# happyxtt/CNNs_SLFP_quantization

Hardware: AMD Instinct MI355X
Metric: images/sec at batch 256, MobileNetV1 SLFP<3,4> ImageNet-224; % HBM roofline (higher is better)
Workload: dtype f32 (1x1 contraction: fp16 MFMA operands, f32 accumulate); 1 GPU; mobilenetv1_imagenet224: all 27 Conv2d_Q layers, SLFP<3,4> Qbits=8, NHWC, batch 256 per GPU as 2 concurrent image groups of 128 on 2 HIP streams, inputs resident in HBM; batch_per_gpu=256, global_batch=256, parallelism=batch-sharded x1, one-time RCCL broadcast of the u8 weight codes, pointwise_mfma=pw_mfma_f16x1

## Files before the change

cnns_slfp_quantization_amd/_lib.py:

```python
import ctypes
import os

_HERE = os.path.dirname(os.path.abspath(__file__))
LIB_PATH = os.path.join(_HERE, "libslfp_hip.so")

OK, ERR_BAD_ARG, ERR_SHAPE, ERR_UNSUPPORTED, ERR_ALIGNMENT, ERR_HIP = 0, -1, -2, -3, -4, -5
FMT_ACT8, FMT_W8, FMT_SFP7, FMT_EXT = 0, 1, 2, 4
LAYOUT_NCHW, LAYOUT_NHWC = 0, 1
BWD_DENSE = 1
MFMA_DEFAULT, MFMA_F16X1, MFMA_F16X3 = 0, 1, 3
OPT_SGD, OPT_DSGD, OPT_SSGD = 0, 1, 2
LAYEROUT_LUT_BYTES = 4928

SYMBOLS = (
    "slfp_version", "slfp_last_error", "slfp_device_count",
    "slfp_encode_f32", "slfp_decode_f32", "slfp_quantize_f32", "slfp_quantize_layerout_f32", "slfp_absmax_f32",
    "slfp_conv2d_out_shape", "slfp_conv2d_kernel_name", "slfp_conv2d_wprep_bytes",
    "slfp_conv2d_prepare_weights", "slfp_conv2d_prepare_weights_codes", "slfp_conv2d_workspace_bytes", "slfp_conv2d_fwd", "slfp_conv2d_fwd_post",
    "slfp_linear_workspace_bytes", "slfp_linear_fwd", "slfp_linear_prepare_weights", "slfp_linear_fwd_prepared",
    "slfp_nchw_to_nhwc_f32", "slfp_nhwc_to_nchw_f32", "slfp_debug_div_mismatches",
    "slfp_debug_enc_mismatches", "slfp_enc_table_ok", "slfp_dwpw_supported", "slfp_dwpw_fwd",
    "slfp_conv2d_codes_supported", "slfp_conv2d_fwd_codes", "slfp_conv2d_fwd_codes_ws", "slfp_maxpool2d_codes", "slfp_debug_code_mismatches", "slfp_debug_reload_switches",
    "slfp_debug_enc_hl_mismatches", "slfp_sgd_step_f32", "slfp_debug_dw3x3_variant", "slfp_debug_dense_variant", "slfp_debug_pw_variant",
    "slfp_conv2d_bwd_supported", "slfp_conv2d_bwd_kernel_name", "slfp_conv2d_bwd_workspace_bytes", "slfp_conv2d_bwd",
    "slfp_conv2d_bwd_supported_ex", "slfp_conv2d_bwd_kernel_name_ex", "slfp_conv2d_bwd_workspace_bytes_ex", "slfp_conv2d_bwd_ex",
    "slfp_conv2d_res_supported", "slfp_conv2d_fwd_res",
    "slfp_conv2d_codes_slice_supported", "slfp_conv2d_fwd_codes_slice", "slfp_maxpool2d_codes_ex", "slfp_maxpool2d_out_shape",
    "slfp_conv2d_entry_supported", "slfp_conv2d_fwd_entry",
    "slfp_conv2d_res_codes_supported", "slfp_conv2d_fwd_res_codes",
    "slfp_layerout_lut_classes", "slfp_layerout_lut_values", "slfp_layerout_lut_index", "slfp_conv2d_codes_lut_supported",
    "slfp_conv2d_fwd_codes_lut", "slfp_debug_layerout_lut_mismatches",
    "slfp_dwpw_codes_supported", "slfp_dwpw_fwd_codes",
    "slfp_linear_fc_supported", "slfp_linear_fc_workspace_bytes", "slfp_linear_fwd_fc", "slfp_debug_linear_fc_tiles",
    "slfp_global_avgpool_supported", "slfp_global_avgpool_f32",
    "slfp_debug_dw3x3_instance", "slfp_debug_code_relu_mismatches",
)


class ConvDesc(ctypes.Structure):
    _fields_ = [
        ("n", ctypes.c_int64), ("c_in", ctypes.c_int64), ("h", ctypes.c_int64), ("w", ctypes.c_int64),
        ("c_out", ctypes.c_int64), ("kh", ctypes.c_int64), ("kw", ctypes.c_int64),
        ("stride_h", ctypes.c_int32), ("stride_w", ctypes.c_int32), ("pad_h", ctypes.c_int32),
        ("pad_w", ctypes.c_int32), ("dil_h", ctypes.c_int32), ("dil_w", ctypes.c_int32),
        ("groups", ctypes.c_int32), ("x_layout", ctypes.c_int32), ("y_layout", ctypes.c_int32),
        ("qbits", ctypes.c_int32), ("ka", ctypes.c_float), ("kw_scale", ctypes.c_float),
        ("mfma_passes", ctypes.c_int32), ("reserved", ctypes.c_int32),
    ]


# ... 30 lines not shown
    dp = ctypes.POINTER(ConvDesc)
    sigs = {
        "slfp_version": (ci, []),
        "slfp_last_error": (ctypes.c_char_p, []),
        "slfp_device_count": (ci, []),
        "slfp_encode_f32": (ci, [vp, vp, sz, cf, ci, vp]),
        "slfp_decode_f32": (ci, [vp, vp, sz, ci, vp]),
        "slfp_quantize_f32": (ci, [vp, vp, sz, cf, ci, vp]),
        "slfp_quantize_layerout_f32": (ci, [vp, vp, sz, vp]),
        "slfp_absmax_f32": (ci, [vp, sz, vp, vp]),
        "slfp_conv2d_out_shape": (ci, [dp, ctypes.POINTER(i64), ctypes.POINTER(i64)]),
        "slfp_conv2d_kernel_name": (ctypes.c_char_p, [dp]),
        "slfp_debug_dw3x3_variant": (ctypes.c_char_p, [dp, ci]),
        "slfp_debug_dw3x3_instance": (ctypes.c_char_p, [dp, ctypes.POINTER(ConvIo), ci, ci, ci]),
        "slfp_debug_code_relu_mismatches": (ci, [cf, ci, vp, vp]),
        "slfp_debug_dense_variant": (ctypes.c_char_p, [dp, ci]),
        "slfp_debug_pw_variant": (ctypes.c_char_p, [dp, ctypes.POINTER(ConvIo), ci, ci, i64]),
        "slfp_conv2d_wprep_bytes": (sz, [dp]),
        "slfp_conv2d_prepare_weights": (ci, [dp, vp, vp, vp, vp]),
        "slfp_conv2d_prepare_weights_codes": (ci, [dp, vp, vp, vp, vp]),
        "slfp_conv2d_workspace_bytes": (sz, [dp]),
        "slfp_conv2d_fwd": (ci, [dp, vp, vp, vp, vp, vp, vp, vp]),
        "slfp_conv2d_fwd_post": (ci, [dp, vp, vp, vp, vp, vp, ci, vp, vp, vp, vp]),
        "slfp_linear_workspace_bytes": (sz, [i64, i64, i64]),
        "slfp_linear_fwd": (ci, [vp, vp, vp, vp, i64, i64, i64, cf, cf, ci, ci, vp, vp]),
        "slfp_linear_prepare_weights": (ci, [vp, vp, i64, i64, cf, ci, ci, vp]),
        "slfp_linear_fwd_prepared": (ci, [vp, vp, vp, vp, i64, i64, i64, cf, cf, ci, ci, vp]),
        "slfp_nchw_to_nhwc_f32": (ci, [vp, vp, i64, i64, i64, i64, vp]),
        "slfp_nhwc_to_nchw_f32": (ci, [vp, vp, i64, i64, i64, i64, vp]),
        "slfp_debug_div_mismatches": (ci, [cf, vp, vp]),
# ... 66 lines not shown
```

cnns_slfp_quantization_amd/csrc/conv_abi.hip:

```cpp
#include <cstring>
#include "slfp_device.hpp"
#include "slfp_codes.hpp"
#include "slfp_layerout_lut.hpp"
#include "slfp_host.hpp"

namespace slfp {

static size_t round256(size_t b) { return (b + 255) & ~(size_t)255; }

static int make_plan_core(const slfp_conv2d_desc* d, ConvPlan* plan) {
    if (!d || !plan) return fail(SLFP_ERR_BAD_ARG, "conv2d: null descriptor");
    if (d->n <= 0 || d->c_in <= 0 || d->h <= 0 || d->w <= 0 || d->c_out <= 0 || d->kh <= 0 || d->kw <= 0)
        return fail(SLFP_ERR_SHAPE, "conv2d: non-positive size");
    if (d->stride_h <= 0 || d->stride_w <= 0 || d->dil_h <= 0 || d->dil_w <= 0 || d->pad_h < 0 || d->pad_w < 0)
        return fail(SLFP_ERR_SHAPE, "conv2d: bad stride/dilation/padding");
    if (d->groups <= 0 || d->c_in % d->groups || d->c_out % d->groups)
        return fail(SLFP_ERR_SHAPE, "conv2d: groups=%d does not divide C_in=%lld / C_out=%lld", d->groups,
                    (long long)d->c_in, (long long)d->c_out);
    if (d->qbits != 8 && d->qbits != 7)
        return fail(SLFP_ERR_BAD_ARG, "conv2d: qbits must be 8 (SLFP<3,4>) or 7 (SFP<3,3>), got %d", d->qbits);
    if ((d->x_layout != SLFP_LAYOUT_NCHW && d->x_layout != SLFP_LAYOUT_NHWC) ||
        (d->y_layout != SLFP_LAYOUT_NCHW && d->y_layout != SLFP_LAYOUT_NHWC))
        return fail(SLFP_ERR_BAD_ARG, "conv2d: unknown layout");
    if (!(d->ka > 0.f) || !(d->kw_scale > 0.f)) return fail(SLFP_ERR_BAD_ARG, "conv2d: Ka and Kw must be > 0");
// ... 237 lines not shown

const char* slfp_debug_dw3x3_instance(const slfp_conv2d_desc* d, const slfp_conv2d_io* io, int has_bias, int post_flags, int has_post) {
    return dw3x3_instance(d, io, has_bias != 0, post_flags, has_post != 0);
}

const char* slfp_debug_dense_variant(const slfp_conv2d_desc* d, int x_codes) {
    ConvPlan p;
    if (make_plan(d, &p) != SLFP_OK) return "none";
    return dense_variant_name(*d, p, x_codes != 0);
}

const char* slfp_debug_pw_variant(const slfp_conv2d_desc* d, const slfp_conv2d_io* io, int has_res, int has_res_codes, int64_t y_ld) {
    return pw_variant(d, io, has_res != 0, has_res_codes != 0, y_ld);
}

size_t slfp_conv2d_wprep_bytes(const slfp_conv2d_desc* d) {
    ConvPlan p;
    if (make_plan(d, &p) != SLFP_OK) return 0;
    return p.wprep_bytes;
}

static int prepare_weights(const char* fn, const slfp_conv2d_desc* d, const void* w, void* wprep, float* weight_q_oihw, void* stream,
                           bool codes) {
    ConvPlan p;
    const int rc = make_plan(d, &p);
    if (rc != SLFP_OK) return rc;
    if (!w || !wprep) return fail(SLFP_ERR_BAD_ARG, "%s: null pointer", fn);
    if (!aligned16(wprep)) return fail(SLFP_ERR_ALIGNMENT, "%s: wprep must be 16-byte aligned", fn);
    return launch_prepare_weights(*d, p, reinterpret_cast<const float*>(w), wprep, weight_q_oihw, as_stream(stream), codes);
}
// ... 572 lines not shown
```

cnns_slfp_quantization_amd/csrc/conv_direct.hip:

```cpp
#include "slfp_device.hpp"
#include "slfp_enc.hpp"
#include "slfp_codes.hpp"
#include "slfp_layerout_lut.hpp"
#include "slfp_host.hpp"
#include "slfp_epilogue.hpp"

namespace slfp {

constexpr int kDirThreads = 256;
constexpr int kDirTH = 8, kDirTW = 8, kDirOC = 64;

struct DirParams {
    int N, H, W, C, O, KH, KW;
    int sh, sw, ph, pw, dh, dw;
    int groups, Cg, Og, Ho, Wo;
    int tiles_h, tiles_w, oc_chunks;
    int CC, IH, IW;
    ScaleDiv sd;
    float s1, s2;
    PostOp post;
    uint32_t nblocks;
};

template <int FMT>
// ... 91 lines not shown
        float* dst = y + (((size_t)n * p.Ho + goh) * p.Wo + gow) * p.O + o0;
        if (o_vec) {
            *reinterpret_cast<float4*>(dst) = make_float4(r4[0], r4[1], r4[2], r4[3]);
        } else {
#pragma unroll
            for (int r = 0; r < 4; ++r)
                if (r < n_o) dst[r] = r4[r];
        }
    }
}


constexpr int kStemTH = 8, kStemTW = 16;

struct StemParams {
    int N, H, W, C, O, KH, KW;
    int s, ph, pw;
    int Ho, Wo, tiles_h, tiles_w;
    int IH, IWC;
    int l4_shift;
    int P;
    int step_h, step_j;
    ScaleDiv sd;
    float s1, s2;
    PostOp post;
    uint32_t nblocks;
    EncArgs enc;
    EncArgsCompact enc_out;
    int sgn, fmt_out;
};

template <int FMT>
__global__ __launch_bounds__(256) void k_stem(const float* __restrict__ x, const float* __restrict__ wq,
                                              const float* __restrict__ bias, float* __restrict__ y, const StemParams p) {
    extern __shared__ __attribute__((aligned(16))) unsigned char smem[];
    uint32_t* sT = reinterpret_cast<uint32_t*>(smem);
    float* sW = reinterpret_cast<float*>(smem + 64);
    const int n_w = p.KH * p.KW * p.C * p.O;
    float* tile = sW + ((n_w + 3) & ~3);
    lut_fill<FMT>(sT);
    for (int i = threadIdx.x * 4; i < n_w; i += 256 * 4)
// ... 258 lines not shown
}

template <bool YC, bool LUTQ = false>
__global__ __launch_bounds__(256) void k_stem_mx(const float* __restrict__ x, const float* __restrict__ wq,
                                                 const float* __restrict__ bias, float* __restrict__ y, const StemParams p) {
    constexpr int KH = 3, KW = 3, C = 3, S = 2, O = 32, TH = 16;
    constexpr int IH = (TH - 1) * S + KH, IWC = ((kStemTW - 1) * S + KW) * C;
    constexpr int N_IN = IH * IWC, U = (N_IN + 255) / 256;
    typedef float f32x4m __attribute__((ext_vector_type(4)));
    __shared__ __attribute__((aligned(16))) float tile[N_IN + 1];
    __shared__ __attribute__((aligned(16))) uint32_t sT[2 * (kEncEntries + 1)];
    static_assert(!LUTQ || YC, "the table epilogue belongs to the code-writing forms");
    __shared__ __attribute__((aligned(16))) unsigned char senc[LUTQ ? kLayeroutLutBytes : (YC ? ((kEncEntries * 8 + 15) & ~15) : 16)];
    constexpr int SP = 36;
    __shared__ __attribute__((aligned(16))) float stg[YC ? 4 : 4 * 16 * SP];
    enc_fill<256>(reinterpret_cast<uint2*>(sT), p.enc);
    if constexpr (LUTQ) layerout_lut_fill<256>(senc, enc_carried_ptr(p.enc_out));
    else if constexpr (YC) enc_fill_compact<256>(reinterpret_cast<uint2*>(senc), p.enc_out);
    if (threadIdx.x == 0) tile[N_IN] = 0.f;

    uint32_t b = xcd_remap(blockIdx.x, p.nblocks);
    const int tw = b % p.tiles_w; b /= p.tiles_w;
    const int th = b % p.tiles_h; b /= p.tiles_h;
    const int n = b;
    const int h_in0 = th * TH * S - p.ph, w_in0 = tw * kStemTW * S - p.pw;

    const int lane = threadIdx.x & 63, wave = threadIdx.x >> 6;
    const int px = lane & 15, kq = lane >> 4;
    float wa[7][2];
#pragma unroll
    for (int ks = 0; ks < 7; ++ks) {
        const int k = 4 * ks + kq;
#pragma unroll
        for (int t = 0; t < 2; ++t) wa[ks][t] = k < KH * KW * C ? wq[k * O + 8 * (px >> 2) + 4 * t + (px & 3)] : 0.f;
    }
    uint32_t koff[7];
#pragma unroll
    for (int ks = 0; ks < 7; ++ks) {
        const int k = 4 * ks + kq;
        koff[ks] = (uint32_t)((k / (KW * C)) * IWC + (k % (KW * C))) * 4u;
    }
    __syncthreads();

    {
        constexpr int Q = (IWC + 1 + 3) / 4;
        constexpr int N4 = IH * Q, U4 = (N4 + 255) / 256;
        const float* xn = x + (size_t)n * p.H * p.W * C;
        const int rowf = p.W * C;
        const int s0 = w_in0 * C - 1;
        const __amdgpu_buffer_rsrc_t rs = __builtin_amdgcn_make_buffer_rsrc(const_cast<float*>(xn), 0, (uint32_t)p.H * p.W * C * 4u, 0x00020000);
        uint32_t vo[U4];
        typedef float f32x4l __attribute__((ext_vector_type(4)));
        f32x4l v[U4];
#pragma unroll
        for (int u = 0; u < U4; ++u) {
            const int idx = threadIdx.x + u * 256;
            const int ih = idx / Q, q = idx - ih * Q;
            const int gh = h_in0 + ih, f0 = s0 + 4 * q;
            const bool ok = idx < N4 && (unsigned)gh < (unsigned)p.H && f0 >= 0 && f0 < rowf;
            vo[u] = ok ? (uint32_t)(gh * rowf + f0) * 4u : 0xFFFFFFF0u;
            asm volatile("" : "+v"(vo[u]));
        }
#pragma unroll
        for (int u = 0; u < U4; ++u) v[u] = __builtin_bit_cast(f32x4l, __builtin_amdgcn_raw_buffer_load_b128(rs, vo[u], 0, 0));
        const unsigned char* tb = reinterpret_cast<const unsigned char*>(sT);
#pragma unroll
        for (int u = 0; u < U4; ++u) {
            const int idx = threadIdx.x + u * 256;
            const int ih = idx / Q, q = idx - ih * Q;
            const float4 xv = make_float4(v[u][0], v[u][1], v[u][2], v[u][3]);
            const float4 qv = enc4_f32(xv, p.enc.r1, p.enc.lo, p.enc.hi, tb);
            const float qs[4] = {qv.x, qv.y, qv.z, qv.w};
            float* trow = tile + ih * IWC + 4 * q - 1;
#pragma unroll
            for (int e = 0; e < 4; ++e)
                if (idx < N4 && 4 * q + e >= 1 && 4 * q + e - 1 < IWC) trow[e] = qs[e];
        }
    }
    __syncthreads();
// ... 100 lines not shown
    p.P = kStemTH / (groups / kStemTW);
    p.step_h = 256 / p.IWC; p.step_j = 256 % p.IWC;
    p.sd = make_scale_div(d.ka); p.s1 = plan.s1; p.s2 = plan.s2;
    const size_t n_w = (size_t)p.KH * p.KW * C * O;
    const size_t lds = 64 + (((n_w + 3) & ~(size_t)3) + (size_t)p.IH * p.IWC) * sizeof(float);
    if (lds > 64 * 1024) return 1;
    const int64_t nblocks = (int64_t)p.N * p.tiles_h * p.tiles_w;
    if (nblocks > 0x7FFFFFFF) return 1;
    p.nblocks = (uint32_t)nblocks;
    if (p.KH == 3 && p.KW == 3 && C == 3 && p.s == 2 && O == 32 && (int64_t)p.H * p.W * C < (1ll << 30)) {
        if (const EncArgs* t = act_table(d.ka, plan.fmt_act, kEncF32)) {
            p.enc = *t;
            constexpr int TH = 16;
            p.tiles_h = (int)ceil_div(p.Ho, TH);
            p.nblocks = (uint32_t)((int64_t)p.N * p.tiles_h * p.tiles_w);
            const bool mx = !switches().stem_old && (p.W * C) % 4 == 0;
            if (mx && !(io && io->y_codes)) {
                hipLaunchKernelGGL((k_stem_mx<false>), dim3(p.nblocks), dim3(256), 0, stream, x, wq_hwio, bias, y, p);
                return check_launch("slfp stem conv kernel (3x3x3 s2 -> 32, float32 MFMA)");
            }
            if (io && io->lut) {
                if (!io->y_codes || !post.scale) return fail(SLFP_ERR_BAD_ARG, "stem (codes): the table epilogue needs code output and post_scale / post_shift");
                p.enc_out.valid = 0;
                enc_carry_ptr(p.enc_out, io->lut);
                p.sgn = 1;
                p.fmt_out = io->y_fmt;
                if (mx) hipLaunchKernelGGL((k_stem_mx<true, true>), dim3(p.nblocks), dim3(256), 0, stream, x, wq_hwio, bias, y, p);
                else hipLaunchKernelGGL((k_stem_fixed<kFmtAct8, 3, 3, 3, 2, 32, true, TH, true, true>), dim3(p.nblocks), dim3(256), 0, stream, x, wq_hwio, bias, y, p);
                return check_launch("slfp stem conv kernel (3x3x3 s2 -> 32, table epilogue)");
            }
// ... 75 lines not shown
```

cnns_slfp_quantization_amd/csrc/conv_dw2.hip:

```cpp
#include <cstdlib>
#include "slfp_device.hpp"
#include "slfp_enc.hpp"
#include "slfp_host.hpp"

namespace slfp {

constexpr int kDw2Threads = 256;
constexpr int kDw2Tab = (kEncEntries * 8 + 15) & ~15;
constexpr uint32_t kOob = 0xFFFFFFF0u;

struct Dw2Params {
    int N, H, W, C, Ho, Wo;
    int tiles_h, tiles_w, cgroups;
    int pad;
    uint32_t ntiles;
    uint32_t nblocks;
    float ka, kw;
    int nt_out;
    PostOp post;
    EncArgs enc;
};

typedef float f32x4 __attribute__((ext_vector_type(4)));

__device__ __forceinline__ __amdgpu_buffer_rsrc_t make_rsrc(const void* base, uint32_t bytes) {
    return __builtin_amdgcn_make_buffer_rsrc(const_cast<void*>(base), 0, bytes, 0x00020000);
}

template <int S, int TH, int TW, bool POST>
__global__ __launch_bounds__(kDw2Threads, 4) void k_dw3x3_tile(const float* __restrict__ x, const float* __restrict__ wq,
                                                               float* __restrict__ y, const Dw2Params p) {
    constexpr int IH = (TH - 1) * S + 3, IW = (TW - 1) * S + 3;
    static_assert(IW <= 16 && IH <= 16, "halo tile is at most 16 x 16 pixel slots");
    constexpr int NI = (IH + 1) / 2;
    constexpr int ROWB = 16 * 32 * 4;

    __shared__ __attribute__((aligned(16))) unsigned char smem[kDw2Tab + 2 * NI * ROWB];
    unsigned char* tile = smem + kDw2Tab;
    enc_fill<kDw2Threads>(reinterpret_cast<uint2*>(smem), p.enc);
    const float r1 = p.enc.r1, lo = p.enc.lo, hi = p.enc.hi;

    const uint32_t lb = xcd_remap(blockIdx.x, p.nblocks);
    const int cg = (int)(lb % (uint32_t)p.cgroups);
    const uint32_t t = lb / (uint32_t)p.cgroups;

    const int c4 = threadIdx.x & 7, slot = threadIdx.x >> 3;
    const int c = cg * 32 + c4 * 4;
    const int iw = slot & 15, ihh = slot >> 4;

    f32x4 wt[9];
#pragma unroll
    for (int k = 0; k < 9; ++k) wt[k] = *reinterpret_cast<const f32x4*>(wq + (size_t)k * p.C + c);
    f32x4 psc = {1.f, 1.f, 1.f, 1.f}, psh = {0.f, 0.f, 0.f, 0.f};
    if constexpr (POST) {
        psc = *reinterpret_cast<const f32x4*>(p.post.scale + c);
        psh = *reinterpret_cast<const f32x4*>(p.post.shift + c);
    }

    const int colslot = (S == 2) ? ((iw & 1) * 8 + (iw >> 1)) : iw;
    const uint32_t lds_w = (uint32_t)((ihh * 16 + colslot) * 128 + c4 * 16);
    const bool col_live = iw < IW;
    constexpr int CW = TW > 8 ? 16 : 8, RPI = 32 / CW, NO = (TH + RPI - 1) / RPI;
    const int ow = slot & (CW - 1), ohb = slot / CW;
    const bool ocol_live = ow < TW;
    const uint32_t lds_r0 = (uint32_t)(((ohb * S) * 16 + ow) * 128 + c4 * 16);
    const uint32_t out_rel0 = (uint32_t)((ohb * p.Wo + ow) * p.C + c) * 4u;
    const uint32_t out_step = (uint32_t)(RPI * p.Wo * p.C) * 4u;
    const uint32_t img_in_bytes = (uint32_t)p.H * p.W * p.C * 4u, img_out_bytes = (uint32_t)p.Ho * p.Wo * p.C * 4u;
    const uint32_t tiles_per_img = (uint32_t)(p.tiles_h * p.tiles_w);

    const uint32_t n = t / tiles_per_img, tr = t - n * tiles_per_img;
    const int th = (int)(tr / (uint32_t)p.tiles_w), tw = (int)(tr - (uint32_t)th * p.tiles_w);

    f32x4 v[NI];
    {
        const __amdgpu_buffer_rsrc_t rs = make_rsrc(x + (size_t)n * p.H * p.W * p.C, img_in_bytes);
        const int gw = tw * TW * S - p.pad + iw;
        const int gh0 = th * TH * S - p.pad + ihh;
        const bool w_ok = col_live && (unsigned)gw < (unsigned)p.W;
        const uint32_t off0 = (uint32_t)((gh0 * p.W + gw) * p.C + c) * 4u;
        const uint32_t step = (uint32_t)(2 * p.W * p.C) * 4u;
        uint32_t voff[NI];
#pragma unroll
        for (int i = 0; i < NI; ++i) {
            bool ok = w_ok && (unsigned)(gh0 + 2 * i) < (unsigned)p.H;
            if (2 * i + 1 >= IH) ok = ok && ihh == 0;
            voff[i] = ok ? off0 + (uint32_t)i * step : kOob;
            asm volatile("" : "+v"(voff[i]));
        }
#pragma unroll
        for (int i = 0; i < NI; ++i)
            v[i] = __builtin_bit_cast(f32x4, __builtin_amdgcn_raw_buffer_load_b128(rs, voff[i], 0, (SLFP_NT_DW & 1) ? 2 : 0));
    }
    __syncthreads();

    bool any_nan = false;
#pragma unroll
    for (int i = 0; i < NI; ++i) {
        const float4 xi = make_float4(v[i][0], v[i][1], v[i][2], v[i][3]);
        any_nan |= enc_has_nan4(xi);
        *reinterpret_cast<float4*>(tile + lds_w + (uint32_t)i * 2u * ROWB) = enc4_f32_raw(xi, r1, lo, hi, smem);
    }
    if (__builtin_expect(any_nan, 0)) {
#pragma unroll
        for (int i = 0; i < NI; ++i)
#pragma unroll
            for (int e = 0; e < 4; ++e)
                if (v[i][e] != v[i][e]) reinterpret_cast<uint32_t*>(tile + lds_w + (uint32_t)i * 2u * ROWB)[e] = kBitsQNaN;
    }
// ... 51 lines not shown
    const Dw2Sel s = dw2_select(d, post);
    if (s.s == 2) return s.post ? "tile/s2/post" : "tile/s2/plain";
    return s.post ? "tile/s1/post" : "tile/s1/plain";
}

int launch_dw3x3_tile(const slfp_conv2d_desc& d, const ConvPlan& plan, const float* x, const float* wq9c,
                      const PostOp& post, float* y, hipStream_t stream) {
    Dw2Params p;
    const Dw2Sel sel = dw2_select(d, post);
    p.post = post;
    p.N = (int)d.n; p.H = (int)d.h; p.W = (int)d.w; p.C = (int)d.c_in;
    p.Ho = (int)plan.h_out; p.Wo = (int)plan.w_out;
    const int S = sel.s;
    const int TH = S == 2 ? 7 : 14, TW = TH;
    p.tiles_h = (int)ceil_div(p.Ho, TH);
    p.tiles_w = (int)ceil_div(p.Wo, TW);
    p.cgroups = p.C / 32;
    p.pad = d.pad_h;
    const int64_t ntiles = (int64_t)p.N * p.tiles_h * p.tiles_w;
    if (ntiles * p.cgroups > 0x7FFFFFFF) return fail(SLFP_ERR_UNSUPPORTED, "dw3x3: grid too large");
    p.ntiles = (uint32_t)ntiles;
    p.nblocks = (uint32_t)(ntiles * p.cgroups);
    p.ka = d.ka; p.kw = d.kw_scale;
    {
        const int64_t min_mb = switches().dw_nt_min_mb;
        p.nt_out = ((SLFP_NT_DW & 2) && (int64_t)p.N * p.Ho * p.Wo * p.C * 4 >= (min_mb << 20)) ? 1 : 0;
    }
    p.enc = *act_table(d.ka, plan.fmt_act, kEncF32);
#define SLFP_DW2(SS, TT) \
    do { if (sel.post) hipLaunchKernelGGL((k_dw3x3_tile<SS, TT, TT, true>), dim3(p.nblocks), dim3(kDw2Threads), 0, stream, x, wq9c, y, p); \
         else hipLaunchKernelGGL((k_dw3x3_tile<SS, TT, TT, false>), dim3(p.nblocks), dim3(kDw2Threads), 0, stream, x, wq9c, y, p); } while (0)
    if (S == 2) SLFP_DW2(2, 7);
    else SLFP_DW2(1, 14);
#undef SLFP_DW2
    return check_launch("slfp dw3x3 (tile) kernel");
}

// ... 2 lines not shown
```

cnns_slfp_quantization_amd/csrc/conv_dw3.hip:

```cpp
#include "slfp_device.hpp"
#include "slfp_enc.hpp"
#include "slfp_host.hpp"

namespace slfp {

constexpr int kDwrThreads = 256;
constexpr int kDwrWaves = kDwrThreads / 64;
constexpr int kDwrTab = (kEncEntries * 8 + 15) & ~15;
constexpr int kDwrTile = 7;

struct DwrParams {
    int N, H, W, C, Ho, Wo, pad;
    int cgs;
    int tiles_h, tiles_w;
    uint32_t ntasks;
    uint32_t nblocks;
    float ka, kw;
    int nt_out;
    PostOp post;
    EncArgs enc;
};

typedef float f32x4 __attribute__((ext_vector_type(4)));
typedef unsigned int u32x4r __attribute__((ext_vector_type(4)));

template <int TH, bool POST>
__global__ __launch_bounds__(kDwrThreads, 4) void k_dw3x3_rows(const float* __restrict__ x, const float* __restrict__ wq,
                                                               float* __restrict__ y, const DwrParams p) {
    constexpr int S = 2, TW = kDwrTile;
    constexpr int NR = (TH - 1) * S + 3;
    constexpr int RING = 3 + S;

    __shared__ __attribute__((aligned(16))) unsigned char smem[kDwrTab];
    enc_fill<kDwrThreads>(reinterpret_cast<uint2*>(smem), p.enc);
    const float r1 = p.enc.r1, lo = p.enc.lo, hi = p.enc.hi;

    uint32_t t = xcd_remap(blockIdx.x, p.nblocks) * kDwrWaves + (uint32_t)__builtin_amdgcn_readfirstlane((int)(threadIdx.x >> 6));
    const bool valid = t < p.ntasks;
    t = valid ? t : p.ntasks - 1;
    const int cg = (int)(t % (uint32_t)p.cgs); t /= (uint32_t)p.cgs;
    const int tw = (int)(t % (uint32_t)p.tiles_w); t /= (uint32_t)p.tiles_w;
    const int th = (int)(t % (uint32_t)p.tiles_h);
    const int n = (int)(t / (uint32_t)p.tiles_h);
    const int lane = (int)(threadIdx.x & 63), g = lane >> 3;
    const int c = cg * 32 + (lane & 7) * 4;

    f32x4 wt[9];
#pragma unroll
    for (int k = 0; k < 9; ++k) wt[k] = *reinterpret_cast<const f32x4*>(wq + (uint32_t)(k * p.C + c));
    f32x4 psc = {1.f, 1.f, 1.f, 1.f}, psh = {0.f, 0.f, 0.f, 0.f};
    if constexpr (POST) {
        psc = *reinterpret_cast<const f32x4*>(p.post.scale + c);
        psh = *reinterpret_cast<const f32x4*>(p.post.shift + c);
    }

    const uint32_t img_in = (uint32_t)(p.H * p.W * p.C) * 4u, img_out = (uint32_t)(p.Ho * p.Wo * p.C) * 4u;
    const __amdgpu_buffer_rsrc_t rs = __builtin_amdgcn_make_buffer_rsrc(const_cast<float*>(x + (size_t)n * (img_in / 4u)), 0, img_in, 0x00020000);
    const __amdgpu_buffer_rsrc_t ry = __builtin_amdgcn_make_buffer_rsrc(y + (size_t)n * (img_out / 4u), 0, img_out, 0x00020000);

    const int ih0 = valid ? th * TH * S - p.pad : -0x40000000;
    const int ow = tw * TW + g, iw0 = ow * S - p.pad;
    const uint32_t rstep = (uint32_t)(p.W * p.C) * 4u;
    const uint32_t rowb = (uint32_t)ih0 * rstep + (uint32_t)c * 4u;
    uint32_t coff[2];
    coff[0] = (unsigned)iw0 < (unsigned)p.W ? (uint32_t)(iw0 * p.C) * 4u : 0x40000000u;
    coff[1] = (g < TW && (unsigned)(iw0 + 1) < (unsigned)p.W) ? (uint32_t)((iw0 + 1) * p.C) * 4u : 0x40000000u;
    const int nb_addr = ((lane + 8) & 63) * 4;

    f32x4 win[RING][3];
    auto request = [&](const int j) {
        const uint32_t roff = (unsigned)(ih0 + j) < (unsigned)p.H ? rowb + (uint32_t)j * rstep : 0x80000000u;
#pragma unroll
        for (int k = 0; k < 2; ++k)
// ... 34 lines not shown
#pragma unroll
                for (int k = 0; k < 2; ++k)
#pragma unroll
                    for (int e = 0; e < 4; ++e)
                        if (nan_mask >> (((j - j0) * 2 + k) * 4 + e) & 1u) win[j % RING][k][e] = __uint_as_float(kBitsQNaN);
        }
#pragma unroll
        for (int j = j0; j < j0 + nj; ++j)
#pragma unroll
            for (int e = 0; e < 4; ++e)
                win[j % RING][2][e] = __int_as_float(__builtin_amdgcn_ds_bpermute(nb_addr, __float_as_int(win[j % RING][0][e])));
    };

#pragma unroll
    for (int j = 0; j < RING && j < NR; ++j) request(j);

    const int oh0 = th * TH;
    const uint32_t ostep = (uint32_t)(p.Wo * p.C) * 4u;
    const uint32_t ocol = (valid && g < TW && ow < p.Wo) ? (uint32_t)((oh0 * p.Wo + ow) * p.C + c) * 4u : 0x80000000u;

    __syncthreads();

    quantize(0, 3 - S);
#pragma unroll
    for (int r = 0; r < TH; ++r) {
        quantize(r * S + 3 - S, S);
        f32x4 acc = {0.f, 0.f, 0.f, 0.f};
#pragma unroll
        for (int kh = 0; kh < 3; ++kh) {
#pragma unroll
            for (int kw = 0; kw < 3; ++kw) {
                const f32x4 a = win[(r * S + kh) % RING][kw];
                const f32x4 w = wt[kh * 3 + kw];
#pragma unroll
                for (int e = 0; e < 4; ++e) acc[e] = fmaf(a[e], w[e], acc[e]);
            }
// ... 27 lines not shown

struct DwrSel { bool post; };
static DwrSel dwr_select(const PostOp& post) { return DwrSel{post.scale != nullptr}; }

const char* dw3x3_rows_name(const slfp_conv2d_desc& d, const ConvPlan& plan, const PostOp& post) {
    return dwr_select(post).post ? "rows/post" : "rows/plain";
}

int launch_dw3x3_rows(const slfp_conv2d_desc& d, const ConvPlan& plan, const float* x, const float* wq9c,
                      const PostOp& post, float* y, hipStream_t stream) {
    DwrParams p;
    const DwrSel sel = dwr_select(post);
    p.post = post;
    p.N = (int)d.n; p.H = (int)d.h; p.W = (int)d.w; p.C = (int)d.c_in;
    p.Ho = (int)plan.h_out; p.Wo = (int)plan.w_out; p.pad = d.pad_h;
    p.cgs = p.C / 32;
    p.tiles_h = (int)ceil_div(p.Ho, kDwrTile);
    p.tiles_w = (int)ceil_div(p.Wo, kDwrTile);
    const int64_t ntasks = (int64_t)p.N * p.tiles_h * p.tiles_w * p.cgs;
    if (ntasks > 0x7FFFFFFF) return fail(SLFP_ERR_UNSUPPORTED, "dw3x3 (rows): grid too large");
    p.ntasks = (uint32_t)ntasks;
    p.nblocks = (uint32_t)ceil_div(ntasks, kDwrWaves);
    p.ka = d.ka; p.kw = d.kw_scale;
    p.nt_out = ((SLFP_NT_DW & 2) && (int64_t)p.N * p.Ho * p.Wo * p.C * 4 >= (switches().dw_nt_min_mb << 20)) ? 1 : 0;
    p.enc = *act_table(d.ka, plan.fmt_act, kEncF32);
    if (sel.post) hipLaunchKernelGGL((k_dw3x3_rows<kDwrTile, true>), dim3(p.nblocks), dim3(kDwrThreads), 0, stream, x, wq9c, y, p);
    else hipLaunchKernelGGL((k_dw3x3_rows<kDwrTile, false>), dim3(p.nblocks), dim3(kDwrThreads), 0, stream, x, wq9c, y, p);
    return check_launch("slfp dw3x3 (rows) kernel");
}

}
```

cnns_slfp_quantization_amd/csrc/slfp_enc.hpp:

```cpp
#pragma once
#include <hip/hip_runtime.h>
#include <stdint.h>

namespace slfp {

constexpr int kEncEntries = 257;
constexpr uint32_t kEncNever = 0x7FC00000u;

constexpr int kEncF32 = 0;
constexpr int kEncF16P = 1;
constexpr int kEncF16LO = 3;

struct EncArgs {
    float r1, lo, hi;
    uint32_t valid;
    uint2 e[kEncEntries];
};

template <int NT>
__device__ __forceinline__ void enc_fill(uint2* sTab, const EncArgs& a) {
    for (int i = threadIdx.x; i < kEncEntries; i += NT) sTab[i] = a.e[i];
}

constexpr int kEncCompact = 146;
struct EncArgsCompact {
    float r1, lo, hi;
    uint32_t valid;
    uint2 e[kEncCompact];
};

inline EncArgsCompact enc_compact(const EncArgs& a) {
    EncArgsCompact c;
    c.r1 = a.r1; c.lo = a.lo; c.hi = a.hi; c.valid = a.valid;
    for (int i = 0; i < kEncCompact; ++i) c.e[i] = a.e[i < 96 ? 160 + i : i - 96];
    return c;
}
// ... 137 lines not shown
```

cnns_slfp_quantization_amd/csrc/slfp_host.hpp:

```cpp
#pragma once
#include <hip/hip_runtime.h>
#include <stdint.h>
#include <stddef.h>
#include <cmath>
#include <cstring>
#include <cstdlib>
#include "../../include/slfp.h"
#include "slfp_device.hpp"
#include "slfp_enc.hpp"

namespace slfp {

void set_error(const char* fmt, ...);
int fail(int code, const char* fmt, ...);
int check_launch(const char* what);

int raise_lds_limit(const void* fn, size_t lds_bytes);

inline hipStream_t as_stream(void* s) { return reinterpret_cast<hipStream_t>(s); }
inline bool aligned16(const void* p) { return (reinterpret_cast<uintptr_t>(p) & 15u) == 0; }
inline int64_t ceil_div(int64_t a, int64_t b) { return (a + b - 1) / b; }

inline bool scale_div_ok(float d) { return std::isfinite(d) && d >= 1e-30f && d <= 1e30f; }

// ... 125 lines not shown

bool stem_small_applicable(const slfp_conv2d_desc& d, int passes);
int stem_small_tiles(const slfp_conv2d_desc& d);
int launch_stem_small(const slfp_conv2d_desc& d, const ConvPlan& p, const float* x, const void* wblob,
                      const float* bias, const PostOp& post, float* y, hipStream_t stream);
bool stem_small_codes_applicable(const slfp_conv2d_desc& d, const ConvPlan& p, int post_flags);
int launch_stem_small_io(const slfp_conv2d_desc& d, const ConvPlan& p, const float* x, const void* wblob, const float* bias,
                         const PostOp& post, void* y_any, const CodeIo& io, hipStream_t stream);

__device__ __forceinline__ uint32_t xcd_remap(uint32_t bid, uint32_t nblocks) {
    const uint32_t xcd = bid & 7u, slot = bid >> 3;
    const uint32_t q = nblocks >> 3, r = nblocks & 7u;
    const uint32_t base = xcd < r ? xcd * (q + 1u) : r * (q + 1u) + (xcd - r) * q;
    return base + slot;
}

}
```

include/slfp.h:

```cpp
#ifndef SLFP_H_
#define SLFP_H_

#include <stddef.h>
#include <stdint.h>

#ifdef __cplusplus
extern "C" {
#endif

#define SLFP_ABI_VERSION 1

#define SLFP_OK 0
#define SLFP_ERR_BAD_ARG (-1)
#define SLFP_ERR_SHAPE (-2)
#define SLFP_ERR_UNSUPPORTED (-3)
#define SLFP_ERR_ALIGNMENT (-4)
#define SLFP_ERR_HIP (-5)

#define SLFP_FMT_ACT8 0
#define SLFP_FMT_W8 1
#define SLFP_FMT_SFP7 2
#define SLFP_FMT_EXT 4

#define SLFP_LAYOUT_NCHW 0
// ... 126 lines not shown
                             const slfp_conv2d_io* io, int has_bias, int relu);
size_t slfp_linear_fc_workspace_bytes(int64_t batch, int64_t in_f, int64_t out_f, const slfp_conv2d_io* io);
int slfp_linear_fwd_fc(const void* x, const void* wprep, const float* bias, void* y, int64_t batch, int64_t in_f,
                       int64_t out_f, float ka, float kw_scale, int qbits, int mfma_passes,
                       const slfp_conv2d_io* io, int relu, void* workspace, void* stream);
int slfp_debug_linear_fc_tiles(int n_tiles, int row_tiles);

int slfp_global_avgpool_supported(int64_t n, int64_t h, int64_t w, int64_t c, int x_layout, const slfp_conv2d_io* io);
int slfp_global_avgpool_f32(const float* x, void* y, int64_t n, int64_t h, int64_t w, int64_t c, int x_layout, int relu,
                            const slfp_conv2d_io* io, void* stream);

int slfp_debug_div_mismatches(float scale_div, unsigned long long* out2, void* stream);

int slfp_debug_enc_mismatches(float scale_div, int fmt, unsigned long long* out2, void* stream);
int slfp_debug_enc_hl_mismatches(float scale_div, int fmt, unsigned long long* out1, void* stream);
int slfp_enc_table_ok(float scale_div, int fmt);

#define SLFP_OPT_SGD 0
#define SLFP_OPT_DSGD 1
#define SLFP_OPT_SSGD 2
typedef struct slfp_sgd_hparams {
    int32_t rule, qbits;
    float lr, momentum, damp_alpha, weight_decay;
    int32_t nesterov, reserved;
} slfp_sgd_hparams;
int slfp_sgd_step_f32(const slfp_sgd_hparams* h, size_t ntensors, float* const* param, float* const* grad,
                      float* const* momentum_buf, const int64_t* numel, const uint8_t* first_step, void* stream);

int slfp_conv2d_bwd_supported(const slfp_conv2d_desc* d);
const char* slfp_conv2d_bwd_kernel_name(const slfp_conv2d_desc* d);
// ... 19 lines not shown
```

Baseline: 132,800 images/sec.

## Issue input loads before table fill; fastdiv block decode in stem and depthwise kernels

```diff
diff --git a/cnns_slfp_quantization_amd/_lib.py b/cnns_slfp_quantization_amd/_lib.py
--- a/cnns_slfp_quantization_amd/_lib.py
+++ b/cnns_slfp_quantization_amd/_lib.py
@@ -33,7 +33,7 @@
     "slfp_dwpw_codes_supported", "slfp_dwpw_fwd_codes",
     "slfp_linear_fc_supported", "slfp_linear_fc_workspace_bytes", "slfp_linear_fwd_fc", "slfp_debug_linear_fc_tiles",
     "slfp_global_avgpool_supported", "slfp_global_avgpool_f32",
-    "slfp_debug_dw3x3_instance", "slfp_debug_code_relu_mismatches",
+    "slfp_debug_dw3x3_instance", "slfp_debug_code_relu_mismatches", "slfp_debug_fastdiv_mismatches",
 )
 
 
@@ -94,6 +94,7 @@
         "slfp_debug_dw3x3_variant": (ctypes.c_char_p, [dp, ci]),
         "slfp_debug_dw3x3_instance": (ctypes.c_char_p, [dp, ctypes.POINTER(ConvIo), ci, ci, ci]),
         "slfp_debug_code_relu_mismatches": (ci, [cf, ci, vp, vp]),
+        "slfp_debug_fastdiv_mismatches": (ctypes.c_ulonglong, [ctypes.c_uint32, ctypes.c_uint32, ctypes.c_uint32]),
         "slfp_debug_dense_variant": (ctypes.c_char_p, [dp, ci]),
         "slfp_debug_pw_variant": (ctypes.c_char_p, [dp, ctypes.POINTER(ConvIo), ci, ci, i64]),
         "slfp_conv2d_wprep_bytes": (sz, [dp]),
diff --git a/cnns_slfp_quantization_amd/csrc/conv_abi.hip b/cnns_slfp_quantization_amd/csrc/conv_abi.hip
--- a/cnns_slfp_quantization_amd/csrc/conv_abi.hip
+++ b/cnns_slfp_quantization_amd/csrc/conv_abi.hip
@@ -275,6 +275,14 @@
     return pw_variant(d, io, has_res != 0, has_res_codes != 0, y_ld);
 }
 
+unsigned long long slfp_debug_fastdiv_mismatches(uint32_t d, uint32_t n_lo, uint32_t n_hi) {
+    if (d == 0 || d >= 0x80000000u || n_hi > 0x80000000u) return ~0ull;
+    const FastDiv f = make_fastdiv(d);
+    unsigned long long bad = 0;
+    for (uint32_t n = n_lo; n < n_hi; ++n) bad += fastdiv(n, f) != n / d;
+    return bad;
+}
+
 size_t slfp_conv2d_wprep_bytes(const slfp_conv2d_desc* d) {
     ConvPlan p;
     if (make_plan(d, &p) != SLFP_OK) return 0;
diff --git a/cnns_slfp_quantization_amd/csrc/conv_direct.hip b/cnns_slfp_quantization_amd/csrc/conv_direct.hip
--- a/cnns_slfp_quantization_amd/csrc/conv_direct.hip
+++ b/cnns_slfp_quantization_amd/csrc/conv_direct.hip
@@ -129,8 +129,11 @@
 constexpr int kStemTH = 8, kStemTW = 16;
 
 struct StemParams {
-    int N, H, W, C, O, KH, KW;
-    int s, ph, pw;
+    uint32_t nblocks;
+    FastDiv by_tw, by_th;
+    int H, W, ph, pw;
+    int N, C, O, KH, KW;
+    int s;
     int Ho, Wo, tiles_h, tiles_w;
     int IH, IWC;
     int l4_shift;
@@ -139,7 +142,6 @@
     ScaleDiv sd;
     float s1, s2;
     PostOp post;
-    uint32_t nblocks;
     EncArgs enc;
     EncArgsCompact enc_out;
     int sgn, fmt_out;
@@ -428,55 +430,63 @@
     __shared__ __attribute__((aligned(16))) unsigned char senc[LUTQ ? kLayeroutLutBytes : (YC ? ((kEncEntries * 8 + 15) & ~15) : 16)];
     constexpr int SP = 36;
     __shared__ __attribute__((aligned(16))) float stg[YC ? 4 : 4 * 16 * SP];
-    enc_fill<256>(reinterpret_cast<uint2*>(sT), p.enc);
-    if constexpr (LUTQ) layerout_lut_fill<256>(senc, enc_carried_ptr(p.enc_out));
-    else if constexpr (YC) enc_fill_compact<256>(reinterpret_cast<uint2*>(senc), p.enc_out);
-    if (threadIdx.x == 0) tile[N_IN] = 0.f;
-
-    uint32_t b = xcd_remap(blockIdx.x, p.nblocks);
-    const int tw = b % p.tiles_w; b /= p.tiles_w;
-    const int th = b % p.tiles_h; b /= p.tiles_h;
-    const int n = b;
+    const uint2 tab = enc_fetch<256, SLFP_ENC_KERNARG_OFF(4, StemParams)>();
+    __builtin_amdgcn_sched_barrier(0);
+
+    const uint32_t b = xcd_remap_sel(blockIdx.x, p.nblocks);
+    const uint32_t b1 = fastdiv(b, p.by_tw);
+    const int tw = (int)(b - b1 * p.by_tw.d);
+    const int n = (int)fastdiv(b1, p.by_th), th = (int)(b1 - (uint32_t)n * p.by_th.d);
     const int h_in0 = th * TH * S - p.ph, w_in0 = tw * kStemTW * S - p.pw;
 
     const int lane = threadIdx.x & 63, wave = threadIdx.x >> 6;
     const int px = lane & 15, kq = lane >> 4;
-    float wa[7][2];
-#pragma unroll
-    for (int ks = 0; ks < 7; ++ks) {
-        const int k = 4 * ks + kq;
-#pragma unroll
-        for (int t = 0; t < 2; ++t) wa[ks][t] = k < KH * KW * C ? wq[k * O + 8 * (px >> 2) + 4 * t + (px & 3)] : 0.f;
-    }
-    uint32_t koff[7];
-#pragma unroll
-    for (int ks = 0; ks < 7; ++ks) {
-        const int k = 4 * ks + kq;
-        koff[ks] = (uint32_t)((k / (KW * C)) * IWC + (k % (KW * C))) * 4u;
-    }
-    __syncthreads();
-
+
+    constexpr int Q = (IWC + 1 + 3) / 4;
+    constexpr int N4 = IH * Q, U4 = (N4 + 255) / 256;
+    typedef float f32x4l __attribute__((ext_vector_type(4)));
+    f32x4l v[U4];
     {
-        constexpr int Q = (IWC + 1 + 3) / 4;
-        constexpr int N4 = IH * Q, U4 = (N4 + 255) / 256;
         const float* xn = x + (size_t)n * p.H * p.W * C;
         const int rowf = p.W * C;
         const int s0 = w_in0 * C - 1;
         const __amdgpu_buffer_rsrc_t rs = __builtin_amdgcn_make_buffer_rsrc(const_cast<float*>(xn), 0, (uint32_t)p.H * p.W * C * 4u, 0x00020000);
         uint32_t vo[U4];
-        typedef float f32x4l __attribute__((ext_vector_type(4)));
-        f32x4l v[U4];
 #pragma unroll
         for (int u = 0; u < U4; ++u) {
             const int idx = threadIdx.x + u * 256;
             const int ih = idx / Q, q = idx - ih * Q;
             const int gh = h_in0 + ih, f0 = s0 + 4 * q;
-            const bool ok = idx < N4 && (unsigned)gh < (unsigned)p.H && f0 >= 0 && f0 < rowf;
+            const bool ok = (idx < N4) & ((unsigned)gh < (unsigned)p.H) & (f0 >= 0) & (f0 < rowf);
             vo[u] = ok ? (uint32_t)(gh * rowf + f0) * 4u : 0xFFFFFFF0u;
             asm volatile("" : "+v"(vo[u]));
         }
 #pragma unroll
         for (int u = 0; u < U4; ++u) v[u] = __builtin_bit_cast(f32x4l, __builtin_amdgcn_raw_buffer_load_b128(rs, vo[u], 0, 0));
+    }
+    __builtin_amdgcn_sched_barrier(0);
+
+    float wa[7][2];
+#pragma unroll
+    for (int ks = 0; ks < 7; ++ks) {
+        const int k = 4 * ks + kq;
+#pragma unroll
+        for (int t = 0; t < 2; ++t) wa[ks][t] = k < KH * KW * C ? wq[k * O + 8 * (px >> 2) + 4 * t + (px & 3)] : 0.f;
+    }
+    enc_store<256>(reinterpret_cast<uint2*>(sT), tab);
+    if constexpr (LUTQ) layerout_lut_fill<256>(senc, enc_carried_ptr(p.enc_out));
+    else if constexpr (YC) enc_fill_compact<256>(reinterpret_cast<uint2*>(senc), p.enc_out);
+    if (threadIdx.x == 0) tile[N_IN] = 0.f;
+    uint32_t koff[7];
+#pragma unroll
+    for (int ks = 0; ks < 7; ++ks) {
+        const int k = 4 * ks + kq;
+        koff[ks] = (uint32_t)((k / (KW * C)) * IWC + (k % (KW * C))) * 4u;
+    }
+    __syncthreads();
+    __builtin_amdgcn_sched_barrier(0);
+
+    {
         const unsigned char* tb = reinterpret_cast<const unsigned char*>(sT);
 #pragma unroll
         for (int u = 0; u < U4; ++u) {
@@ -607,6 +617,8 @@
             constexpr int TH = 16;
             p.tiles_h = (int)ceil_div(p.Ho, TH);
             p.nblocks = (uint32_t)((int64_t)p.N * p.tiles_h * p.tiles_w);
+            p.by_tw = make_fastdiv((uint32_t)p.tiles_w);
+            p.by_th = make_fastdiv((uint32_t)p.tiles_h);
             const bool mx = !switches().stem_old && (p.W * C) % 4 == 0;
             if (mx && !(io && io->y_codes)) {
                 hipLaunchKernelGGL((k_stem_mx<false>), dim3(p.nblocks), dim3(256), 0, stream, x, wq_hwio, bias, y, p);
diff --git a/cnns_slfp_quantization_amd/csrc/conv_dw2.hip b/cnns_slfp_quantization_amd/csrc/conv_dw2.hip
--- a/cnns_slfp_quantization_amd/csrc/conv_dw2.hip
+++ b/cnns_slfp_quantization_amd/csrc/conv_dw2.hip
@@ -10,11 +10,12 @@
 constexpr uint32_t kOob = 0xFFFFFFF0u;
 
 struct Dw2Params {
-    int N, H, W, C, Ho, Wo;
-    int tiles_h, tiles_w, cgroups;
-    int pad;
+    uint32_t nblocks;
+    FastDiv by_cg, by_tiles, by_tw;
+    int H, W, C, pad;
+    int N, Ho, Wo;
+    int tiles_h;
     uint32_t ntiles;
-    uint32_t nblocks;
     float ka, kw;
     int nt_out;
     PostOp post;
@@ -37,40 +38,20 @@
 
     __shared__ __attribute__((aligned(16))) unsigned char smem[kDw2Tab + 2 * NI * ROWB];
     unsigned char* tile = smem + kDw2Tab;
-    enc_fill<kDw2Threads>(reinterpret_cast<uint2*>(smem), p.enc);
-    const float r1 = p.enc.r1, lo = p.enc.lo, hi = p.enc.hi;
-
-    const uint32_t lb = xcd_remap(blockIdx.x, p.nblocks);
-    const int cg = (int)(lb % (uint32_t)p.cgroups);
-    const uint32_t t = lb / (uint32_t)p.cgroups;
+    const uint2 tab = enc_fetch<kDw2Threads, SLFP_ENC_KERNARG_OFF(3, Dw2Params)>();
+    __builtin_amdgcn_sched_barrier(0);
+
+    const uint32_t lb = xcd_remap_sel(blockIdx.x, p.nblocks);
+    const uint32_t t = fastdiv(lb, p.by_cg);
+    const int cg = (int)(lb - t * p.by_cg.d);
+    const uint32_t n = fastdiv(t, p.by_tiles), tr = t - n * p.by_tiles.d;
+    const int th = (int)fastdiv(tr, p.by_tw), tw = (int)(tr - (uint32_t)th * p.by_tw.d);
 
     const int c4 = threadIdx.x & 7, slot = threadIdx.x >> 3;
     const int c = cg * 32 + c4 * 4;
     const int iw = slot & 15, ihh = slot >> 4;
-
-    f32x4 wt[9];
-#pragma unroll
-    for (int k = 0; k < 9; ++k) wt[k] = *reinterpret_cast<const f32x4*>(wq + (size_t)k * p.C + c);
-    f32x4 psc = {1.f, 1.f, 1.f, 1.f}, psh = {0.f, 0.f, 0.f, 0.f};
-    if constexpr (POST) {
-        psc = *reinterpret_cast<const f32x4*>(p.post.scale + c);
-        psh = *reinterpret_cast<const f32x4*>(p.post.shift + c);
-    }
-
-    const int colslot = (S == 2) ? ((iw & 1) * 8 + (iw >> 1)) : iw;
-    const uint32_t lds_w = (uint32_t)((ihh * 16 + colslot) * 128 + c4 * 16);
     const bool col_live = iw < IW;
-    constexpr int CW = TW > 8 ? 16 : 8, RPI = 32 / CW, NO = (TH + RPI - 1) / RPI;
-    const int ow = slot & (CW - 1), ohb = slot / CW;
-    const bool ocol_live = ow < TW;
-    const uint32_t lds_r0 = (uint32_t)(((ohb * S) * 16 + ow) * 128 + c4 * 16);
-    const uint32_t out_rel0 = (uint32_t)((ohb * p.Wo + ow) * p.C + c) * 4u;
-    const uint32_t out_step = (uint32_t)(RPI * p.Wo * p.C) * 4u;
-    const uint32_t img_in_bytes = (uint32_t)p.H * p.W * p.C * 4u, img_out_bytes = (uint32_t)p.Ho * p.Wo * p.C * 4u;
-    const uint32_t tiles_per_img = (uint32_t)(p.tiles_h * p.tiles_w);
-
-    const uint32_t n = t / tiles_per_img, tr = t - n * tiles_per_img;
-    const int th = (int)(tr / (uint32_t)p.tiles_w), tw = (int)(tr - (uint32_t)th * p.tiles_w);
+    const uint32_t img_in_bytes = (uint32_t)p.H * p.W * p.C * 4u;
 
     f32x4 v[NI];
     {
@@ -92,7 +73,30 @@
         for (int i = 0; i < NI; ++i)
             v[i] = __builtin_bit_cast(f32x4, __builtin_amdgcn_raw_buffer_load_b128(rs, voff[i], 0, (SLFP_NT_DW & 1) ? 2 : 0));
     }
+    __builtin_amdgcn_sched_barrier(0);
+
+    f32x4 wt[9];
+#pragma unroll
+    for (int k = 0; k < 9; ++k) wt[k] = *reinterpret_cast<const f32x4*>(wq + (size_t)k * p.C + c);
+    f32x4 psc = {1.f, 1.f, 1.f, 1.f}, psh = {0.f, 0.f, 0.f, 0.f};
+    if constexpr (POST) {
+        psc = *reinterpret_cast<const f32x4*>(p.post.scale + c);
+        psh = *reinterpret_cast<const f32x4*>(p.post.shift + c);
+    }
+    enc_store<kDw2Threads>(reinterpret_cast<uint2*>(smem), tab);
+    const float r1 = p.enc.r1, lo = p.enc.lo, hi = p.enc.hi;
+
+    const int colslot = (S == 2) ? ((iw & 1) * 8 + (iw >> 1)) : iw;
+    const uint32_t lds_w = (uint32_t)((ihh * 16 + colslot) * 128 + c4 * 16);
+    constexpr int CW = TW > 8 ? 16 : 8, RPI = 32 / CW, NO = (TH + RPI - 1) / RPI;
+    const int ow = slot & (CW - 1), ohb = slot / CW;
+    const bool ocol_live = ow < TW;
+    const uint32_t lds_r0 = (uint32_t)(((ohb * S) * 16 + ow) * 128 + c4 * 16);
+    const uint32_t out_rel0 = (uint32_t)((ohb * p.Wo + ow) * p.C + c) * 4u;
+    const uint32_t out_step = (uint32_t)(RPI * p.Wo * p.C) * 4u;
+    const uint32_t img_out_bytes = (uint32_t)p.Ho * p.Wo * p.C * 4u;
     __syncthreads();
+    __builtin_amdgcn_sched_barrier(0);
 
     bool any_nan = false;
 #pragma unroll
@@ -174,13 +178,15 @@
     const int S = sel.s;
     const int TH = S == 2 ? 7 : 14, TW = TH;
     p.tiles_h = (int)ceil_div(p.Ho, TH);
-    p.tiles_w = (int)ceil_div(p.Wo, TW);
-    p.cgroups = p.C / 32;
+    const int tiles_w = (int)ceil_div(p.Wo, TW), cgroups = p.C / 32;
     p.pad = d.pad_h;
-    const int64_t ntiles = (int64_t)p.N * p.tiles_h * p.tiles_w;
-    if (ntiles * p.cgroups > 0x7FFFFFFF) return fail(SLFP_ERR_UNSUPPORTED, "dw3x3: grid too large");
+    const int64_t ntiles = (int64_t)p.N * p.tiles_h * tiles_w;
+    if (ntiles * cgroups > 0x7FFFFFFF) return fail(SLFP_ERR_UNSUPPORTED, "dw3x3: grid too large");
     p.ntiles = (uint32_t)ntiles;
-    p.nblocks = (uint32_t)(ntiles * p.cgroups);
+    p.nblocks = (uint32_t)(ntiles * cgroups);
+    p.by_cg = make_fastdiv((uint32_t)cgroups);
+    p.by_tiles = make_fastdiv((uint32_t)(p.tiles_h * tiles_w));
+    p.by_tw = make_fastdiv((uint32_t)tiles_w);
     p.ka = d.ka; p.kw = d.kw_scale;
     {
         const int64_t min_mb = switches().dw_nt_min_mb;
diff --git a/cnns_slfp_quantization_amd/csrc/conv_dw3.hip b/cnns_slfp_quantization_amd/csrc/conv_dw3.hip
--- a/cnns_slfp_quantization_amd/csrc/conv_dw3.hip
+++ b/cnns_slfp_quantization_amd/csrc/conv_dw3.hip
@@ -10,11 +10,11 @@
 constexpr int kDwrTile = 7;
 
 struct DwrParams {
-    int N, H, W, C, Ho, Wo, pad;
-    int cgs;
-    int tiles_h, tiles_w;
+    uint32_t nblocks;
     uint32_t ntasks;
-    uint32_t nblocks;
+    FastDiv by_cg, by_tw, by_th;
+    int H, W, C, pad;
+    int N, Ho, Wo;
     float ka, kw;
     int nt_out;
     PostOp post;
@@ -32,31 +32,21 @@
     constexpr int RING = 3 + S;
 
     __shared__ __attribute__((aligned(16))) unsigned char smem[kDwrTab];
-    enc_fill<kDwrThreads>(reinterpret_cast<uint2*>(smem), p.enc);
+    const uint2 tab = enc_fetch<kDwrThreads, SLFP_ENC_KERNARG_OFF(3, DwrParams)>();
+    __builtin_amdgcn_sched_barrier(0);
     const float r1 = p.enc.r1, lo = p.enc.lo, hi = p.enc.hi;
 
-    uint32_t t = xcd_remap(blockIdx.x, p.nblocks) * kDwrWaves + (uint32_t)__builtin_amdgcn_readfirstlane((int)(threadIdx.x >> 6));
+    uint32_t t = xcd_remap_sel(blockIdx.x, p.nblocks) * kDwrWaves + (uint32_t)__builtin_amdgcn_readfirstlane((int)(threadIdx.x >> 6));
     const bool valid = t < p.ntasks;
     t = valid ? t : p.ntasks - 1;
-    const int cg = (int)(t % (uint32_t)p.cgs); t /= (uint32_t)p.cgs;
-    const int tw = (int)(t % (uint32_t)p.tiles_w); t /= (uint32_t)p.tiles_w;
-    const int th = (int)(t % (uint32_t)p.tiles_h);
-    const int n = (int)(t / (uint32_t)p.tiles_h);
+    const uint32_t t1 = fastdiv(t, p.by_cg), t2 = fastdiv(t1, p.by_tw);
+    const int cg = (int)(t - t1 * p.by_cg.d), tw = (int)(t1 - t2 * p.by_tw.d);
+    const int n = (int)fastdiv(t2, p.by_th), th = (int)(t2 - (uint32_t)n * p.by_th.d);
     const int lane = (int)(threadIdx.x & 63), g = lane >> 3;
     const int c = cg * 32 + (lane & 7) * 4;
 
-    f32x4 wt[9];
-#pragma unroll
-    for (int k = 0; k < 9; ++k) wt[k] = *reinterpret_cast<const f32x4*>(wq + (uint32_t)(k * p.C + c));
-    f32x4 psc = {1.f, 1.f, 1.f, 1.f}, psh = {0.f, 0.f, 0.f, 0.f};
-    if constexpr (POST) {
-        psc = *reinterpret_cast<const f32x4*>(p.post.scale + c);
-        psh = *reinterpret_cast<const f32x4*>(p.post.shift + c);
-    }
-
     const uint32_t img_in = (uint32_t)(p.H * p.W * p.C) * 4u, img_out = (uint32_t)(p.Ho * p.Wo * p.C) * 4u;
     const __amdgpu_buffer_rsrc_t rs = __builtin_amdgcn_make_buffer_rsrc(const_cast<float*>(x + (size_t)n * (img_in / 4u)), 0, img_in, 0x00020000);
-    const __amdgpu_buffer_rsrc_t ry = __builtin_amdgcn_make_buffer_rsrc(y + (size_t)n * (img_out / 4u), 0, img_out, 0x00020000);
 
     const int ih0 = valid ? th * TH * S - p.pad : -0x40000000;
     const int ow = tw * TW + g, iw0 = ow * S - p.pad;
@@ -121,12 +111,25 @@
 
 #pragma unroll
     for (int j = 0; j < RING && j < NR; ++j) request(j);
-
+    __builtin_amdgcn_sched_barrier(0);
+
+    f32x4 wt[9];
+#pragma unroll
+    for (int k = 0; k < 9; ++k) wt[k] = *reinterpret_cast<const f32x4*>(wq + (uint32_t)(k * p.C + c));
+    f32x4 psc = {1.f, 1.f, 1.f, 1.f}, psh = {0.f, 0.f, 0.f, 0.f};
+    if constexpr (POST) {
+        psc = *reinterpret_cast<const f32x4*>(p.post.scale + c);
+        psh = *reinterpret_cast<const f32x4*>(p.post.shift + c);
+    }
+    enc_store<kDwrThreads>(reinterpret_cast<uint2*>(smem), tab);
+
+    const __amdgpu_buffer_rsrc_t ry = __builtin_amdgcn_make_buffer_rsrc(y + (size_t)n * (img_out / 4u), 0, img_out, 0x00020000);
     const int oh0 = th * TH;
     const uint32_t ostep = (uint32_t)(p.Wo * p.C) * 4u;
     const uint32_t ocol = (valid && g < TW && ow < p.Wo) ? (uint32_t)((oh0 * p.Wo + ow) * p.C + c) * 4u : 0x80000000u;
 
     __syncthreads();
+    __builtin_amdgcn_sched_barrier(0);
 
     quantize(0, 3 - S);
 #pragma unroll
@@ -184,11 +187,12 @@
     p.post = post;
     p.N = (int)d.n; p.H = (int)d.h; p.W = (int)d.w; p.C = (int)d.c_in;
     p.Ho = (int)plan.h_out; p.Wo = (int)plan.w_out; p.pad = d.pad_h;
-    p.cgs = p.C / 32;
-    p.tiles_h = (int)ceil_div(p.Ho, kDwrTile);
-    p.tiles_w = (int)ceil_div(p.Wo, kDwrTile);
-    const int64_t ntasks = (int64_t)p.N * p.tiles_h * p.tiles_w * p.cgs;
+    const int cgs = p.C / 32, tiles_h = (int)ceil_div(p.Ho, kDwrTile), tiles_w = (int)ceil_div(p.Wo, kDwrTile);
+    const int64_t ntasks = (int64_t)p.N * tiles_h * tiles_w * cgs;
     if (ntasks > 0x7FFFFFFF) return fail(SLFP_ERR_UNSUPPORTED, "dw3x3 (rows): grid too large");
+    p.by_cg = make_fastdiv((uint32_t)cgs);
+    p.by_tw = make_fastdiv((uint32_t)tiles_w);
+    p.by_th = make_fastdiv((uint32_t)tiles_h);
     p.ntasks = (uint32_t)ntasks;
     p.nblocks = (uint32_t)ceil_div(ntasks, kDwrWaves);
     p.ka = d.ka; p.kw = d.kw_scale;
diff --git a/cnns_slfp_quantization_amd/csrc/slfp_enc.hpp b/cnns_slfp_quantization_amd/csrc/slfp_enc.hpp
--- a/cnns_slfp_quantization_amd/csrc/slfp_enc.hpp
+++ b/cnns_slfp_quantization_amd/csrc/slfp_enc.hpp
@@ -20,6 +20,24 @@
 template <int NT>
 __device__ __forceinline__ void enc_fill(uint2* sTab, const EncArgs& a) {
     for (int i = threadIdx.x; i < kEncEntries; i += NT) sTab[i] = a.e[i];
+}
+
+template <int NT, uint32_t KOFF>
+__device__ __forceinline__ uint2 enc_fetch() {
+    static_assert(NT == 256 && KOFF % 8 == 0, "one 8-byte entry per thread");
+    typedef unsigned int u32x2e __attribute__((ext_vector_type(2)));
+    const char* seg = (const char*)__builtin_amdgcn_kernarg_segment_ptr();
+    const __amdgpu_buffer_rsrc_t rs = __builtin_amdgcn_make_buffer_rsrc(const_cast<char*>(seg) + KOFF + __builtin_offsetof(EncArgs, e), 0,
+                                                                        (uint32_t)sizeof(uint2) * kEncEntries, 0x00020000);
+    const u32x2e e = __builtin_amdgcn_raw_buffer_load_b64(rs, threadIdx.x * 8u, 0, 0);
+    return make_uint2(e[0], e[1]);
+}
+#define SLFP_ENC_KERNARG_OFF(NPTR, P) ((uint32_t)(((NPTR) * 8 + alignof(P) - 1) / alignof(P) * alignof(P) + __builtin_offsetof(P, enc)))
+template <int NT>
+__device__ __forceinline__ void enc_store(uint2* sTab, const uint2 e) {
+    static_assert(NT == 256, "one entry per thread");
+    sTab[threadIdx.x] = e;
+    sTab[threadIdx.x == 0 ? 256 : threadIdx.x] = e;
 }
 
 constexpr int kEncCompact = 146;
diff --git a/cnns_slfp_quantization_amd/csrc/slfp_host.hpp b/cnns_slfp_quantization_amd/csrc/slfp_host.hpp
--- a/cnns_slfp_quantization_amd/csrc/slfp_host.hpp
+++ b/cnns_slfp_quantization_amd/csrc/slfp_host.hpp
@@ -163,5 +163,28 @@
     const uint32_t base = xcd < r ? xcd * (q + 1u) : r * (q + 1u) + (xcd - r) * q;
     return base + slot;
 }
+__device__ __forceinline__ uint32_t xcd_remap_sel(uint32_t bid, uint32_t nblocks) {
+    const uint32_t xcd = bid & 7u, q = nblocks >> 3, r = nblocks & 7u;
+    return xcd * q + (xcd < r ? xcd : r) + (bid >> 3);
+}
+
+struct FastDiv {
+    uint32_t d, mul, shift;
+};
+inline FastDiv make_fastdiv(uint32_t d) {
+    FastDiv f;
+    f.d = d;
+    f.shift = 0;
+    while ((1ull << f.shift) < d) ++f.shift;
+    f.mul = (uint32_t)(((1ull << (31 + f.shift)) + d - 1) / d);
+    return f;
+}
+__host__ __device__ __forceinline__ uint32_t fastdiv(uint32_t n, const FastDiv& f) {
+#if defined(__HIP_DEVICE_COMPILE__)
+    return __umulhi(n << 1, f.mul) >> f.shift;
+#else
+    return (uint32_t)(((uint64_t)(n << 1) * f.mul) >> 32) >> f.shift;
+#endif
+}
 
 }
diff --git a/include/slfp.h b/include/slfp.h
--- a/include/slfp.h
+++ b/include/slfp.h
@@ -164,6 +164,7 @@
 
 int slfp_debug_enc_mismatches(float scale_div, int fmt, unsigned long long* out2, void* stream);
 int slfp_debug_enc_hl_mismatches(float scale_div, int fmt, unsigned long long* out1, void* stream);
+unsigned long long slfp_debug_fastdiv_mismatches(uint32_t d, uint32_t n_lo, uint32_t n_hi);
 int slfp_enc_table_ok(float scale_div, int fmt);
 
 #define SLFP_OPT_SGD 0
```

Measured after the change: 133,200 images/sec (median of 6 runs). Within noise of the previous version (+0.3%).
